# astrodeepnet/debvader

Hardware: AMD Instinct MI355X
Metric: galaxy stamps/sec (train fwd+bwd+Adam) 59x59x6 (higher is better)
Workload: dtype f32; 1 GPU; BASELINE configs[1]: 6-band 59x59 stamps, batch=256 per GPU, latent_dim=32, filters [32,64,128,256], fp32, stage-1 VAE train step; global_batch=256, per_gpu_batch=256, parallelism=dp1

## Files before the change

debvader_amd/csrc/common.h:

```cpp
#pragma once
#include <hip/hip_runtime.h>
#include <stdint.h>
#include <stddef.h>
#include <memory>
#include <utility>

namespace dv {

enum : int {
  OK = 0,
  E_INVALID = -1,
  E_HIP = -2,
  E_NOMEM = -3,
  E_RCCL = -4,
  E_STATE = -5,
  E_NODEVICE = -6,
};

void set_error(const char* fmt, ...);
int hip_fail(hipError_t e, const char* what, const char* file, int line);

#define DV_HIP(call)                                                     \
  do {                                                                   \
    hipError_t e__ = (call);                                             \
// ... 161 lines not shown
                                 const float* eps, double* res2_f = nullptr);
int launch_scene_fields_copy(double* dst_dev, const double* src_dev, const int* fptr_dev, int M, long felems, hipStream_t s);
long scene_field_mse_blocks(long felems);
int launch_scene_field_mse(const double* a_dev, const double* b_dev, const int* fptr_dev, int M, long felems,
                           double* part_dev, double* out_dev, hipStream_t s);
int launch_scene_eps_norm(const float* eps, const float* loc, int n, int cs, int nb, double* out_dev, hipStream_t s);
int launch_scene_center_mse(const double* field_dev, int F, int nb, const int* starts_dev, const float* loc, int n, int cs,
                            double* out_dev, hipStream_t s, const int* sfield_dev, int f0);
size_t scene_frac_coef_doubles(int cs, int nb, int planes);
size_t scene_frac_obj_bytes(size_t n);
int launch_scene_places(const double* dist_dev, const double* shifts_dev, int n, int F, int cs, void* objs_dev,
                        hipStream_t s);
int launch_scene_composite_frac(double* mean_f, double* std_f, double* res_f, int F, int nb, const float* loc,
                                const float* scale, const void* objs_dev, int n, int cs, hipStream_t s, const int* fptr_dev,
                                int f0, const int32_t* sfield_h, long obase, double* eps_f, const float* eps,
                                double* res2_f, double* coef_dev);
int scene_extract(const double* field_h, int F, int nb, const int32_t* starts_h, int N, int cs, double* out_h,
                  hipStream_t s);
int scene_composite(double* field_h, int F, int nb, const double* stamps_h, const double* pos_h, int N, int cs,
                    double sign, hipStream_t s);
int scene_fit_shifts(const double* field_h, int F, const double* stamps_h, int N, int cs, const double* dist_h,
                     double bound, int max_iter, double* shifts_h, double* objective_h, int32_t* iters_h,
                     int32_t* status_h, hipStream_t s);
int scene_fit_shifts_fields(const double* fields_h, int M, int F, const double* stamps_h, const int64_t* field_ptr, int N,
                            int cs, const double* dist_h, double bound, int max_iter, double* shifts_h, double* objective_h,
                            int32_t* iters_h, int32_t* status_h, size_t budget_bytes, hipStream_t s);
struct PosfitPlan;
int posfit_plan_create(int F, int cs, int N, const double* dist_h, const double* shifts_h, double bound, int max_iter,
                       PosfitPlan** out);
void posfit_plan_destroy(PosfitPlan* p);
struct PosfitPlanFree { void operator()(PosfitPlan* p) const { posfit_plan_destroy(p); } };
using PosfitPlanOwner = std::unique_ptr<PosfitPlan, PosfitPlanFree>;
int posfit_plan_layout(PosfitPlan* p, int a, int b, int max_n, const int32_t* sfield, int f0, int stamp0);
void posfit_plan_rebase(PosfitPlan* p, int a, int b, int f0);
int posfit_plan_launch_count(const PosfitPlan* p);
long posfit_plan_work_doubles(const PosfitPlan* p);
size_t posfit_plan_geom_bytes(size_t n);
int posfit_plan_upload(PosfitPlan* p, hipStream_t s);
int posfit_plan_run(const PosfitPlan* p, int l0, int l1, const double* img_dev, const double* total_sq_dev,
                    const double* stamps_dev, double* work_dev, double* shifts_dev, double* objective_dev, int* iters_dev,
                    int* status_dev, hipStream_t s);
int launch_posfit_total_sq(const double* img_dev, int nfields, long elems, double* out_dev, hipStream_t s);
int launch_posfit_band_f64(const double* src_dev, long npix, int nb, int band, double* dst_dev, hipStream_t s);
int launch_posfit_band_f32(const float* src_dev, long npix, int nb, int band, double* dst_dev, hipStream_t s);
int measure_check(const char* who, int cs, int nb, int band, double sigma0, double tol, int max_iter);
int launch_measure(const float* mean_dev, const float* stddev_dev, int n, int cs, int nb, int band, double sigma0,
                   double tol, int max_iter, double* flux_dev, double* flux_err_dev, double* shape_dev, int* iters_dev,
                   int* status_dev, hipStream_t s);
int scene_measure(const float* mean_h, const float* stddev_h, int64_t N, int cs, int nb, int band, double sigma0, double tol,
                  int max_iter, double* flux_h, double* flux_err_h, double* shape_h, int32_t* iters_h, int32_t* status_h,
                  int64_t chunk, hipStream_t s);
struct McScratch { double *flux, *shape; int *iters, *status; };
struct McState {
  double *flux_mean, *flux_std, *shape_mean, *shape_std;
  int* n_ok;
  double *sample_flux, *sample_shape;
  int* sample_status;
};
int launch_measure_mc_samples(const float* pass_dev, int rows, int cs, int nb, int band, double sigma0, double tol,
                              int max_iter, const McScratch& w, hipStream_t s);
int launch_measure_mc_fold(const McScratch& w, int n, int reps, int k0, int S, int nb, const McState& st, int64_t row0,
                           hipStream_t s);
int scene_measure_mc(const float* samples_h, int S, int64_t N, int cs, int nb, int band, double sigma0, double tol,
                     int max_iter, const McState& out_h, int64_t chunk, hipStream_t s);
int blend_check(const char* who, int cs, int nb, int band);
int launch_blend_child(const float* stamps_dev, const double* shape_dev, const int* status_dev, const int* places_dev, int n,
                       int cs, int nb, int band, int F, double* blend_dev, int* npix_dev, hipStream_t s);
int launch_blend_parent(const double* shape_dev, const int* status_dev, const int* places_dev, const int* sfield_dev, int f0,
                        int n, int cs, int nb, int band, int F, const double* model_dev, const double* data_dev,
                        double* blend_dev, hipStream_t s);
int launch_blend_composite_mean(double* mean_f, int F, int nb, const float* loc, const int* places_dev, int n, int cs,
                                const int* fptr_dev, int f0, int fy0, int nfields, long obase, hipStream_t s);
int launch_blend_set(const double* shape_dev, const int* status_dev, const int* places_dev, const int* sfield_dev, int n, int cs,
                     int nb, int band, int F, const double* mean_dev, const double* base_dev, const double* final_dev,
                     double* sums_dev, hipStream_t s);
int scene_blend(const float* stamps_h, const double* shape_h, const int32_t* status_h, const int32_t* places_h,
                const int64_t* field_ptr, int64_t N, int cs, int nb, int band, const double* model_h, const double* data_h,
                int M, int F, double* blend_h, int32_t* npix_h, int64_t chunk, int64_t gmax, hipStream_t s);
int scene_detect(const double* fields_h, int M, int H, int W, double thresh, double cont, int minarea, int nthresh,
                 int back_size, int back_filter, const double* kernel_h, int kh, int kw, int64_t workspace_bytes,
                 int64_t cap, int64_t* n_out, int64_t* offsets_h, double* globalrms_h, int32_t* field_h,
                 int32_t* parent_h, int32_t* npix_h, double* peak_h, double* flux_h, double* x_h, double* y_h,
                 double* back_h, double* rms_h, double* D_h, int32_t* labels_h, hipStream_t s);
struct DetectDevSrc {
  const double* fields_dev;
  int nb, band;
  const int32_t* which_h;
};
int scene_detect_dev(const DetectDevSrc& src, int M, int H, int W, double thresh, double cont, int minarea, int nthresh,
                     int back_size, int back_filter, const double* kernel_h, int kh, int kw, int64_t workspace_bytes,
                     int64_t cap, int64_t* n_out, int64_t* offsets_h, double* globalrms_h, int32_t* field_h,
                     int32_t* parent_h, int32_t* npix_h, double* peak_h, double* flux_h, double* x_h, double* y_h,
                     hipStream_t s);

struct GStripParams {
  const float* X;
  const float* W;
  float* U;
  float* A;
  const float* bias;
  const float* alpha;
  const float* zero;
  int NB, H, Wd, Cin, Cout;
  unsigned long long tapcode, wtcode;
  int epi;
  int R, patch_floats, strips_per_stamp, nstrips, strips_per_wg;
};
int launch_gconv_strip(GStripParams p, bool nmajor, hipStream_t s);
int launch_gconv_strip8(GStripParams p, hipStream_t s);

struct WinoParams {
  const float* X;
  const float* Ut;
  float* U;
  float* A;
  const float* bias;
  const float* alpha;
  const float* zero;
  int NB, H, Cin, Cout;
  int epi;
  int nbh, nct, NC, groups, items, items_per_wg;
};
struct WinoWDesc {
  const float* W;
  float* Ut;
  int Cin, Cout, nmajor;
  int wtmap[9];
};
struct WinoWgradParams {
  const float* X;
  const float* Y;
  float* part;
  size_t part_capacity;
  const float* zero;
  int NB, H, Cx, Cy;
  int nbh, nkt, nnt, nblocks, S, bps;
};
bool wino_wgrad_supported(int NB, int H, int Cx, int Cy);
size_t wino_wgrad_part_floats(int NB, int H, int Cx, int Cy, int* splits_out);
int launch_wino_wgrad(WinoWgradParams p, float* out, hipStream_t s);
int launch_wino_wgrad_finish(const float* part, float* out, int S, int Cx, int Cy, hipStream_t s);
bool wino_supported(int NB, int H, int Cin, int Cout);
size_t wino_weight_floats(int Cin, int Cout);
int launch_wino_weights(const WinoWDesc* descs_dev, const WinoWDesc* descs_host, int n, hipStream_t s);
int launch_wino_conv(WinoParams p, hipStream_t s);

struct GConvS2Params {
  const float* X;
  const float* W;
  float* U;
  float* A;
  const float* bias;
  const float* alpha;
  int NB, Hin, Win, Cin;
  int Hout, Wout, Cout;
  int Hc, Wc, M;
  int epi;
  int ndh[4], ndw[4];
  int cph[4], cpw[4];
  int wt[4][4];
  unsigned* dbg_out;
};
int launch_gconv_s2(const GConvS2Params& p, hipStream_t s);
void debug_set_gconv_s2_tile(int code);
void debug_set_wino_variant(int v);
void debug_set_gconv_s2_dbg(unsigned* out);

struct WGradParams {
  const float* X;
  const float* Y;
  float* part;
  int NB, Hx, Wx, Cx;
  int Hy, Wy, Cy;
  int Hc, Wc, sx, sy, ph, pw;
  int ntaps;
  TapTab xt;
  int P;
  int rows_total;
  int nsplit;
  int pchunk;
  unsigned div_hw_m, div_hw_s1, div_hw_s2, div_w_m, div_w_s1, div_w_s2;
};
int launch_wgrad(const WGradParams& p, hipStream_t s);
int launch_dense_wgrad_tn(const float* X, int ldx, const float* Y, int ldy, int NB, int I, int J, float* G, int ldg,
                          hipStream_t s);

struct WStripParams {
  const float* X;
  const float* Y;
  float* part;
  size_t part_capacity;
  int NB, Hx, Wx, Hy, Wy;
  int pb;
  const float* zero;
  int R, XR, xs_floats, ys_floats, strips_per_stamp, nstrips, strips_per_wg;
  int dbg;
  const float* U;
  const float* alpha;
  float* dal_part;
  float* db_part;
  size_t dal_capacity, db_capacity;
  long alpha_elems;
  int groups;
  int* groups_out;
};
bool wgrad_strip8_fusable(int Hy, int Wy);
void debug_set_strip(int v);
bool wgrad_strip_supported(int Cx, int Cy, int sx, int ntaps);
int launch_wgrad_strip(const WStripParams& p, int Cx, int Cy, int sx, hipStream_t s, int* nsplit_out);

#define DV_WRED_MAX 24
struct WRedEntry {
  const float* part;
  float* out;
  int nsplit, slab4, ncols4, cpad, creal;
};
struct WRedBatch {
  WRedEntry e[DV_WRED_MAX];
  int count;
};
int launch_reduce_partials_batch(const WRedBatch& b, hipStream_t s);
int launch_reduce_partials(const float* part, float* out, int nsplit, long slab_elems, int ncols, int cpad,
                           int creal, hipStream_t s);

struct HeadParams {
  const float* tpre;
  const float* y;
  const int* idx;
  int first;
  float* dt;
  float* loc;
  float* scale;
  float* part;
  int NB, Hd, H, nb, crop0;
  int ld;
  float sigma_floor;
  float gscale;
  int mse_sample;
  int mse_row0;
  unsigned mse_stream;
  unsigned long long mse_seed;
};
#define DV_MSE_STREAM 0x4D534500u
int launch_head(const HeadParams& p, hipStream_t s, int* nblocks_out);

constexpr int DV_BN_MAXC = 16;
int launch_bn_stats(const float* x, const int* idx, int first, int NB, int HW, int C, float* part, int* nblocks,
                    hipStream_t s);
int launch_reduce_rows_f64(const float* part, int nrows, int ncols, float* out, float scale, hipStream_t s,
                           int ld = 0);
int launch_bn_finalize(const float* sums, float count, int C, const float* gamma, const float* beta,
                       float* moving_mean, float* moving_var, float eps, float momentum, int unbiased,
                       int training, int update_moving, float* bnstate, hipStream_t s);
int launch_bn_apply(const float* x, const int* idx, int first, int NB, int HW, int C, int Cpad, const float* bnstate,
                    float* xn, hipStream_t s);
int launch_prelu_fwd(const float* u, const float* alpha, float* a, long NB, int E, hipStream_t s);
int launch_prelu_bwd(float* da, const float* u, const float* alpha, int NB, int E, int C, int nsplit,
                     float* dalpha_part, float* dbias_part, int* dbias_rows, hipStream_t s);
int launch_colsum(const float* x, long rows, int C, float* part, int* nrows_part, hipStream_t s);
int launch_dense_narrow(const float* x, const float* W, float* out, int NB, int K, int N, hipStream_t s);


struct SamplerParams {
  const float* t;
  float* eps;
  float* z;
  float* kl;
  float* stddev;
  int NB, d;
  int ldt, ldz;
  float diag_shift;
  int gen;
  unsigned long long seed;
  unsigned stream;
  unsigned row0;
  int rep_nb;
  const unsigned long long* seed_ptr;
  const float* slab;
  const float* tbias;
  float* t_out;
  long slab_stride;
  int nslab, lds;
  const float* alpha_in;
  float* ain;
};
int launch_sampler_fwd(const SamplerParams& p, hipStream_t s);
int launch_sampler_bwd(const float* t, const float* eps, const float* z, const float* dz, float* dt, int NB, int d,
                       int ldt, int ldz, float diag_shift, float kls, hipStream_t s);
int launch_sampler_wide_fwd(const SamplerParams& p, hipStream_t s);
int launch_sampler_wide_bwd(const float* t, const float* eps, const float* z, const float* dz, float* dt, int NB, int d,
                            int ldt, int ldz, float diag_shift, float kls, hipStream_t s);

int launch_adam(float* w, float* m, float* v, const float* g, long n, float lr_t, float b1, float b2, float eps,
                hipStream_t s);
int launch_pad_w1(const float* w, const float* gamma, const float* beta, float* wp, int taps, int cin, int cpad,
                  int cout, hipStream_t s);
int launch_bn_conv0_grads(const float* G, const float* w, const float* gamma, const float* beta, float* dW,
                          float* dgamma, float* dbeta, int taps, int cin, int cpad, int cout, hipStream_t s);
int launch_fill(float* p, long n, float v, hipStream_t s);
int launch_normalise(float* x, long n, bool inverse, hipStream_t s);
int launch_welford_update(const float* x, float* mean, float* m2, long n, int k, hipStream_t s);
int launch_welford_finish(float* m2, long n, int count, hipStream_t s);
int launch_welford_update_multi(const float* x, float* mean, float* m2, long n, int reps, int k0, hipStream_t s);
int launch_pad_cols(const float* src, float* dst, int rows, int nsrc, int ndst, hipStream_t s);
int launch_take_cols(const float* src, float* dst, int rows, int nsrc, int ndst, hipStream_t s);
int launch_gather_rows(const float* src, const int* idx, int first, int NB, long row_elems, float* dst,
                       hipStream_t s);


#if defined(__HIPCC__)
__device__ __forceinline__ void dv_dma_exec(unsigned lds, unsigned voff, const void* sbase, unsigned long long mask);
template <bool LAST16>
__device__ __forceinline__ void dv_dma_masked(unsigned lds, unsigned voff, const void* sbase, unsigned long long m_dma,
                                              unsigned vnull, const void* zero) {
// ... 27 lines not shown
```

debvader_amd/csrc/engine.hip:

```cpp
#include <rccl/rccl.h>
#include <math.h>
#include <stdarg.h>
#include <stdio.h>
#include <stdlib.h>
#include <string.h>
#include <unistd.h>

#include <algorithm>
#include <string>
#include <thread>
#include <map>
#include <memory>
#include <mutex>
#include <set>
#include <vector>
#ifdef DV_DEBUG_EXPORTS
#include <functional>
#endif

#include "../../include/debvader_hip.h"
#ifdef DV_DEBUG_EXPORTS
#include "../../include/debvader_hip_debug.h"
#endif
#include <chrono>
// ... 951 lines not shown
  p.X = X;
  p.W = W;
  p.U = U;
  p.A = Aout;
  p.bias = bias;
  p.alpha = alpha;
  p.NB = NB;
  p.Hin = p.Win = Hin;
  p.Cin = Cin;
  p.Hout = p.Wout = Hout;
  p.Cout = Cout;
  p.Hc = p.Wc = Hout;
  p.sin = s;
  p.sout = 1;
  p.ph = p.pw = 0;
  p.M = NB * Hout * Hout;
  p.w_nmajor = nmajor ? 1 : 0;
  p.epi = epi;
  Taps one;
  one.add(0, 0, 0);
  const Taps tp = single_tap ? one : taps_fprop(pb, ksz);
  const bool k3 = single_tap || ksz == 3;
  const double flops = 2.0 * NB * Hout * Hout * tp.n * (double)(W == m->W1p ? m->A.C : Cin) *
                       (double)(W == m->Whp ? 2 * m->A.C : Cout);
  if (k3 && s == 1 && pb == 1 && Hin == Hout && tp.n == 9 && !single_tap && !g_force_v1 && !g_no_special && !(fz && !m->no_fuse)) {
    const int r = wino_conv(m, X, W, nmajor, tp, bias, alpha, U, Aout, epi, NB, Hout, Cin, Cout, flops);
    if (r <= 0) return r;
  }
  if (k3 && Cin == 32 && (Cout == 16 || Cout == 32) && s == 1 && Hin == Hout && Hout >= 8 && Hout <= 64 && tp.n == 9 &&
      !single_tap && !g_force_v1 && !g_no_special && !(fz && !m->no_fuse)) {
    GStripParams g;
    memset(&g, 0, sizeof g);
    g.X = X; g.W = W; g.U = U; g.A = Aout; g.bias = bias; g.alpha = alpha; g.zero = m->zero_page;
    g.NB = NB; g.H = Hout; g.Wd = Hout; g.Cin = Cin; g.Cout = Cout;
    g.tapcode = tp.tapcode; g.wtcode = tp.wtcode; g.epi = epi;
    int r;
    {
      ProfScope ps(m, 0, nullptr, PF_GSTRIP, flops);
      r = launch_gconv_strip(g, nmajor, fwd_stream(m));
      if (r > 0) prof_uncount(m, 0, PF_GSTRIP, flops);
    }
    if (r <= 0) return r;
  }
  if (k3 && Cin == 8 && Cout == 32 && s == 1 && pb == 1 && !nmajor && Hin == Hout && Hout >= 8 && Hout <= 64 && tp.n == 9 &&
      !single_tap && !g_force_v1 && !g_no_special && !fz) {
    GStripParams g;
    memset(&g, 0, sizeof g);
    g.X = X; g.W = W; g.U = U; g.A = Aout; g.bias = bias; g.alpha = alpha; g.zero = m->zero_page;
    g.NB = NB; g.H = Hout; g.Wd = Hout; g.Cin = Cin; g.Cout = Cout; g.epi = epi;
    int r;
    {
      ProfScope ps(m, 0, nullptr, PF_GSTRIP8, flops);
      r = launch_gconv_strip8(g, fwd_stream(m));
      if (r > 0) prof_uncount(m, 0, PF_GSTRIP8, flops);
    }
    if (r <= 0) return r;
  }
  if (single_tap && nmajor && Hin == 1 && Hout == 1 && Cout <= 64 && Cin <= 1024 && epi == 0 && !bias && !fz && !g_force_v1 &&
      !g_no_special) {
    ProfScope ps(m, 2);
    if (exp_skip_small()) return OK;
    return launch_dense_narrow(X, W, U, NB, Cin, Cout, fwd_stream(m));
  }
  const bool ragged_dense = single_tap && Cin > 32 && (Cin & 3) == 0 && (Cin % 32) != 0 && !fz && !g_no_special;
  if ((Cin % 32 == 0 || ragged_dense || ((Cin == 8 || Cin == 16) && Cout <= 32 && !single_tap)) && !g_force_v1 && k3 &&
      tp.legacy) {
    GConv2Params q;
    memset(&q, 0, sizeof q);
    q.X = X; q.W = W; q.U = U; q.A = Aout; q.bias = bias; q.alpha = alpha;
    q.NB = NB; q.Hin = q.Win = Hin; q.Cin = Cin; q.Hout = q.Wout = Hout; q.Cout = Cout;
    q.sin = s; q.sout = 1; q.nclass = 1;
    q.cls[0].Hc = q.cls[0].Wc = Hout; q.cls[0].M = NB * Hout * Hout; q.cls[0].ph = q.cls[0].pw = 0;
    q.cls[0].ntaps = tp.n; q.cls[0].tapcode = tp.tapcode; q.cls[0].wtcode = tp.wtcode;
    q.w_nmajor = nmajor ? 1 : 0; q.epi = epi;
    const long MN = (long)NB * Hout * Hout * Cout;
    const long tiles64 = ((q.cls[0].M + 63) / 64) * (long)((Cout + 63) / 64);
    const int nchunks = tp.n * ((Cin + 31) / 32);
    if (single_tap && tiles64 < 256 && nchunks >= 32 && m->ws4) {
      const size_t ws4_cap = m->ws4_elems / 4;
      float* ws4 = m->ws4 + (size_t)m->lane_id * ws4_cap;
      int ks = (int)std::min<long>(std::min<long>(16, nchunks / 8), (long)(ws4_cap / (size_t)MN));
      if (ks > 1) {
        q.ksplit = ks;
        q.U = ws4;
        q.A = nullptr;
        q.epi = 0;
        {
          ProfScope ps(m, 0, nullptr, PF_GCONV2, flops);
          DV_TRY(launch_gconv2(q, fwd_stream(m)));
        }
        ProfScope ps(m, 2);
        if (exp_skip_small()) return OK;
        return launch_splitk_finish(ws4, ks, MN, Cout, epi >= 1 ? bias : nullptr, epi == 2 ? alpha : nullptr,
                                    (long)Hout * Hout * Cout, U, epi == 2 ? Aout : nullptr, fwd_stream(m));
      }
    }
    if (!fz && !single_tap) {
      const int r = gconv2_small_splitk(m, q, NB, Hout, Cout, nchunks, epi, bias, alpha, U, Aout, flops);
      if (r != 0) return r < 0 ? r : OK;
    }
    long db_rows = 0;
    const bool fuse = fz && !m->no_fuse && fuse_setup(m, q, fz, &db_rows) == OK;
    {
      ProfScope ps(m, 0, nullptr, PF_GCONV2, flops);
      DV_TRY(launch_gconv2(q, fwd_stream(m)));
    }
    if (fuse) {
      if (fused) *fused = true;
      return fuse_finish(m, q, fz, db_rows);
    }
    return OK;
  }
  fill_gconv_common(p, tp, Cin);
  ProfScope ps(m, 0, nullptr, PF_GCONV, flops);
  return launch_gconv(p, fwd_stream(m));
}

static int gconv_dgrad(dv_model* m, const float* X, const float* W, bool nmajor, const float* bias, const float* alpha,
                       float* U, float* Aout, int epi, int NB, int Hs, int Cs, int Ht, int Ct, int s, int pb,
                       const FuseBwd* fz = nullptr, bool* fused = nullptr, int ksz = 3) {
  if (fused) *fused = false;
  const double flops = 2.0 * NB * Hs * Hs * (double)(ksz * ksz) * (double)(W == m->Whp ? 2 * m->A.C : Cs) * (double)Ct;
  const bool k3 = ksz == 3;
  if (k3 && s == 1 && pb == 1 && Hs == Ht && !g_force_v1 && !g_no_special && !(fz && !m->no_fuse)) {
    const Taps tp = taps_dgrad(1, pb, 0, 0);
    if (tp.n == 9) {
      const int r = wino_conv(m, X, W, nmajor, tp, bias, alpha, U, Aout, epi, NB, Ht, Cs, Ct, flops);
      if (r <= 0) return r;
    }
  }
  if (k3 && s == 1 && (Cs == 32 || (Cs == 16 && Ct == 32)) && (Ct == 16 || Ct == 32) && Hs == Ht && Ht >= 8 && Ht <= 64 && !g_force_v1 && !g_no_special &&
      !(fz && !m->no_fuse)) {
    const Taps tp = taps_dgrad(1, pb, 0, 0);
    if (tp.n == 9) {
      GStripParams g;
      memset(&g, 0, sizeof g);
      g.X = X; g.W = W; g.U = U; g.A = Aout; g.bias = bias; g.alpha = alpha; g.zero = m->zero_page;
      g.NB = NB; g.H = Ht; g.Wd = Ht; g.Cin = Cs; g.Cout = Ct;
      g.tapcode = tp.tapcode; g.wtcode = tp.wtcode; g.epi = epi;
      int r;
      {
        ProfScope ps(m, 0, nullptr, PF_GSTRIP, flops);
        r = launch_gconv_strip(g, nmajor, fwd_stream(m));
        if (r > 0) prof_uncount(m, 0, PF_GSTRIP, flops);
      }
      if (r <= 0) return r;
    }
  }
  const bool tiny_splitk = m->tiny_call && NB <= 16 && !fz;
  if (k3 && s == 2 && Cs % 32 == 0 && Ct % 4 == 0 && nmajor && !g_force_v1 && !g_no_special && !(fz && !m->no_fuse) &&
      !tiny_splitk) {
    GConvS2Params q;
    memset(&q, 0, sizeof q);
    q.X = X; q.W = W; q.U = U; q.A = Aout; q.bias = bias; q.alpha = alpha;
    q.NB = NB; q.Hin = q.Win = Hs; q.Cin = Cs; q.Hout = q.Wout = Ht; q.Cout = Ct;
    q.Hc = q.Wc = (Ht + 1) / 2; q.M = NB * q.Hc * q.Wc; q.epi = epi;
    int two = -1, x = 0, kk[2][2] = {{-1, -1}, {-1, -1}};
    bool ok = true;
    for (int ph = 0; ph < 2; ++ph) {
      int n = 0;
      for (int kh = 0; kh < 3; ++kh) {
        const int nh = ph + pb - kh;
        if (nh & 1) continue;
        const int d = nh / 2;
        ++n;
        if (d == 0) kk[ph][0] = kh; else { kk[ph][1] = kh; x = d; two = ph; }
      }
      if (kk[ph][0] < 0 || n > 2) ok = false;
    }
    if (ok && two >= 0 && kk[1 - two][1] < 0) {
      for (int c = 0; c < 4; ++c) {
        q.cph[c] = (c & 2) ? two : 1 - two;
        q.cpw[c] = (c & 1) ? two : 1 - two;
      }
      for (int e = 0; e < 4; ++e) {
        q.ndh[e] = (e & 2) ? x : 0;
        q.ndw[e] = (e & 1) ? x : 0;
        for (int c = 0; c < 4; ++c)
          if ((e & ~c) == 0) q.wt[e][c] = kk[q.cph[c]][(e & 2) ? 1 : 0] * 3 + kk[q.cpw[c]][(e & 1) ? 1 : 0];
      }
      ProfScope ps(m, 0, nullptr, PF_GCONV_S2, flops);
      return launch_gconv_s2(q, fwd_stream(m));
    }
  }
  if (k3 && (Cs % 32 == 0 || ((Cs == 8 || Cs == 16) && Ct <= 32)) && s <= 2 && !g_force_v1) {
    GConv2Params q;
    memset(&q, 0, sizeof q);
    q.X = X; q.W = W; q.U = U; q.A = Aout; q.bias = bias; q.alpha = alpha;
    q.NB = NB; q.Hin = q.Win = Hs; q.Cin = Cs; q.Hout = q.Wout = Ht; q.Cout = Ct;
    q.sin = 1; q.sout = s; q.w_nmajor = nmajor ? 1 : 0; q.epi = epi;
    struct C { int ph, pw, n; } order[4];
    int nc = 0;
    for (int ph = 0; ph < s; ++ph)
      for (int pw = 0; pw < s; ++pw) order[nc++] = {ph, pw, taps_dgrad(s, pb, ph, pw).n};
    std::sort(order, order + nc, [](const C& a, const C& b) { return a.n > b.n; });
    int k = 0;
    for (int i = 0; i < nc; ++i) {
      int hc = (Ht - order[i].ph + s - 1) / s, wc = (Ht - order[i].pw + s - 1) / s;
      if (hc <= 0 || wc <= 0) continue;
      Taps t = taps_dgrad(s, pb, order[i].ph, order[i].pw);
      if (t.n == 0) {
        set_error("empty parity class");
        return E_INVALID;
      }
      GClass2& c = q.cls[k++];
      c.Hc = hc; c.Wc = wc; c.M = NB * hc * wc; c.ph = order[i].ph; c.pw = order[i].pw;
      c.ntaps = t.n; c.tapcode = t.tapcode; c.wtcode = t.wtcode;
    }
    q.nclass = k;
    if (!fz && k >= 1 && Cs % 32 == 0) {
      int maxtaps = 0;
      for (int i = 0; i < k; ++i) maxtaps = std::max(maxtaps, q.cls[i].ntaps);
      const int r = gconv2_small_splitk(m, q, NB, Ht, Ct, maxtaps * (Cs / 32), epi, bias, alpha, U, Aout, flops);
      if (r != 0) return r < 0 ? r : OK;
    }
    long db_rows = 0;
    const bool fuse = fz && !m->no_fuse && fuse_setup(m, q, fz, &db_rows) == OK;
    {
      ProfScope ps(m, 0, nullptr, PF_GCONV2, flops);
      DV_TRY(launch_gconv2(q, fwd_stream(m)));
    }
    if (fuse) {
      if (fused) *fused = true;
      return fuse_finish(m, q, fz, db_rows);
    }
    return OK;
  }
  for (int ph = 0; ph < s; ++ph)
    for (int pw = 0; pw < s; ++pw) {
      int hc = (Ht - ph + s - 1) / s, wc = (Ht - pw + s - 1) / s;
      if (hc <= 0 || wc <= 0) continue;
      Taps t = taps_dgrad(s, pb, ph, pw, ksz);
      GConvParams p;
      memset(&p, 0, sizeof p);
      p.X = X;
      p.W = W;
      p.U = U;
      p.A = Aout;
      p.bias = bias;
      p.alpha = alpha;
      p.NB = NB;
      p.Hin = p.Win = Hs;
      p.Cin = Cs;
      p.Hout = p.Wout = Ht;
      p.Cout = Ct;
      p.Hc = hc;
      p.Wc = wc;
      p.sin = 1;
      p.sout = s;
      p.ph = ph;
      p.pw = pw;
      p.M = NB * hc * wc;
      p.w_nmajor = nmajor ? 1 : 0;
      p.epi = epi;
      fill_gconv_common(p, t, Cs);
      ProfScope ps(m, 0, nullptr, PF_GCONV, flops * t.n / (double)(ksz * ksz));
      DV_TRY(launch_gconv(p, fwd_stream(m)));
    }
  return OK;
}

static int wgrad_impl(dv_model* m, hipStream_t ws, const float* X, int Hx, int Cx, const float* Y, int Hy, int Cy, int NB,
                      int sx, int pb, bool single_tap, float* out, int cpad, int creal, const FuseBwd* fz, int ksz);

static int wgrad(dv_model* m, const float* X, int Hx, int Cx, const float* Y, int Hy, int Cy, int NB, int sx, int pb,
                 bool single_tap, float* out, int cpad, int creal, const FuseBwd* fz = nullptr, bool on_main = false,
                 int ksz = 3) {
  hipStream_t ws = (m->wstream && !on_main) ? m->wstream : m->ctx->stream;
  if (ws != m->ctx->stream) {
    if (!m->main_marked) DV_HIP(hipEventRecord(m->ctx->ev_ready, m->ctx->stream));
    DV_HIP(hipStreamWaitEvent(ws, m->ctx->ev_ready, 0));
  }
  m->main_marked = false;
  return wgrad_impl(m, ws, X, Hx, Cx, Y, Hy, Cy, NB, sx, pb, single_tap, out, cpad, creal, fz, ksz);
}

static int wgrad_impl(dv_model* m, hipStream_t ws, const float* X, int Hx, int Cx, const float* Y, int Hy, int Cy, int NB,
                      int sx, int pb, bool single_tap, float* out, int cpad, int creal, const FuseBwd* fz, int ksz) {
  const bool k3 = ksz == 3;
  {
    static const int exp_all = DV_EXP_SWITCH("DV_EXP_SKIP_WGRAD");
    if (exp_all == 2 && !single_tap && !fz) return OK;
    if (single_tap && exp_skip_dense()) return OK;
  }
  dv_ctx* cx = m->ctx;
  const double wflops = 2.0 * NB * Hy * Hy * (single_tap ? 1.0 : (double)(ksz * ksz)) * (double)(X == m->xn ? m->A.C : Cx) *
                        (double)(out == m->Ghs ? 2 * m->A.C : Cy);
  {
    static const bool onepass = getenv("DV_DENSE_WGRAD_ONEPASS") != nullptr;
    if (single_tap && Hx == 1 && Hy == 1 && sx == 1 && cpad == creal && !fz && !g_force_v1 && !g_no_special && onepass &&
        !(Cx & 1) && !(Cy & 3)) {
      {
        ProfScope ps(m, 1, ws, PF_WGRAD, wflops);
        DV_TRY(launch_dense_wgrad_tn(X, Cx, Y, Cy, NB, Cx, Cy, out, Cy, ws));
      }
      m->ws_last_rs = ws;
      m->ws_last = -1;
      return OK;
    }
  }
  const bool rot = m->wstream && m->wstream != cx->stream && m->arena_reduce && cx->red_stream && m->ev_wk[0];
  const bool per_launch = m->ws_nreg > 3;
  float* part = m->ws1;
  size_t part_cap = m->ws1_elems;
  hipStream_t rs = ws;
  int reg = -1;
  if (rot) {
// ... 4595 lines not shown
```

debvader_amd/csrc/gconv_s2.hip:

```cpp
#include "common.h"
#include <stdlib.h>

namespace dv {

namespace {
constexpr int BKS = 32;
template <int V>
struct IC {
  static constexpr int value = V;
};
__host__ __device__ constexpr int phase_nbr(int ph) { return 3 - ph; }
__host__ __device__ constexpr int nbr_mask(int e) {
  return (e == 0) ? 15 : (e == 1) ? 10 : (e == 2) ? 12 : 8;
}
__host__ __device__ constexpr int popc4(int m) { return (m & 1) + ((m >> 1) & 1) + ((m >> 2) & 1) + ((m >> 3) & 1); }
}

template <int WGM, int WGN, int TMW = 2>
__global__ __launch_bounds__(64 * WGM * WGN) void gconv_s2_kernel(const GConvS2Params p) {
  constexpr int NW = WGM * WGN, NT = 64 * NW;
  constexpr int WMR = 16 * TMW;
  constexpr int BM = WMR * WGM, BN = 32 * WGN;
  constexpr int RP = NT / 8;
  constexpr int AROWS = BM / RP, BROWS = BN / RP;
  constexpr int A_ELEMS = BM * BKS, B_ELEMS = BN * BKS;
  constexpr int STAGE = A_ELEMS + 4 * B_ELEMS;
  constexpr int LDC = 36;
  static_assert(NW * WMR * LDC <= 2 * STAGE, "staging must fit in the operand buffers");

  extern __shared__ __attribute__((aligned(16))) float smem[];
  int* s_in = reinterpret_cast<int*>(smem + 2 * STAGE);
  int* s_nm = s_in + BM;
  int* s_out = s_nm + BM;
  int* s_al = s_out + BM;

  const unsigned long long tl0 = p.dbg_out ? __builtin_amdgcn_s_memrealtime() : 0ull;
  const int tid = threadIdx.x, lane = tid & 63, wave = tid >> 6;
  const int wm0 = (wave / WGN) * WMR, wn0 = (wave % WGN) * 32;
  const int l15 = lane & 15, lg = lane >> 4;

  int bid = blockIdx.x;
  {
    const int nwg = gridDim.x, q8 = nwg >> 3, r8 = nwg & 7, xcd = bid & 7, loc = bid >> 3;
    bid = (xcd < r8 ? xcd * (q8 + 1) : r8 * (q8 + 1) + (xcd - r8) * q8) + loc;
  }
  const int ntn = (p.Cout + BN - 1) / BN;
  const int m0 = (bid / ntn) * BM;
  const int n0 = (bid % ntn) * BN;

  if (tid < BM) {
    const int m = m0 + tid;
    int in_off = 0, nm = 0, out_off = 0, al_off = 0;
    if (m < p.M) {
      const int HW = p.Hc * p.Wc;
      const int nb = m / HW, rem = m - nb * HW;
      const int ii = rem / p.Wc, jj = rem - ii * p.Wc;
      in_off = ((nb * p.Hin + ii) * p.Win + jj) * p.Cin;
#pragma unroll
      for (int e = 0; e < 4; ++e) {
        const int ih = ii + p.ndh[e], iw = jj + p.ndw[e];
        if ((unsigned)ih < (unsigned)p.Hin && (unsigned)iw < (unsigned)p.Win) nm |= 1 << e;
      }
#pragma unroll
      for (int c = 0; c < 4; ++c)
        if (2 * ii + p.cph[c] < p.Hout && 2 * jj + p.cpw[c] < p.Wout) nm |= 16 << c;
      al_off = (2 * ii * p.Wout + 2 * jj) * p.Cout;
      out_off = nb * p.Hout * p.Wout * p.Cout + al_off;
    }
    s_in[tid] = in_off;
    s_nm[tid] = nm;
    s_out[tid] = out_off;
    s_al[tid] = al_off;
  }
  __syncthreads();

  const int kq = tid & 7, r0 = tid >> 3;
  int rin[AROWS];
  unsigned rnm = 0;
#pragma unroll
  for (int i = 0; i < AROWS; ++i) {
    rin[i] = s_in[r0 + RP * i] + kq * 4;
    rnm |= (unsigned)(s_nm[r0 + RP * i] & 15) << (4 * i);
  }
  int wthr[BROWS];
  unsigned wok = 0;
#pragma unroll
  for (int i = 0; i < BROWS; ++i) {
    const int n = n0 + r0 + RP * i;
    const bool ok = n < p.Cout;
    wthr[i] = ok ? n * p.Cin + kq * 4 : 0;
    wok |= (ok ? 1u : 0u) << i;
  }

  f32x4 areg[AROWS];
  f32x4 breg[4][BROWS];
  unsigned amask = 0;
  const int cpt = p.Cin / BKS;
  const int CC = p.Cout * p.Cin;

  auto load_global = [&](auto phase, int cc) {
    constexpr int E = phase_nbr(decltype(phase)::value);
    constexpr int MK = nbr_mask(E);
    const int tapoff = (p.ndh[E] * p.Win + p.ndw[E]) * p.Cin + cc * BKS;
    amask = 0;
#pragma unroll
    for (int i = 0; i < AROWS; ++i) {
      const bool ok = (rnm >> (4 * i + E)) & 1;
      const unsigned off = ok ? (unsigned)(rin[i] + tapoff) : 0u;
      areg[i] = *reinterpret_cast<const f32x4*>(p.X + off);
      amask |= (ok ? 1u : 0u) << i;
    }
#pragma unroll
    for (int c = 0; c < 4; ++c) {
      if ((MK >> c) & 1) {
        const int wbase = p.wt[E][c] * CC + cc * BKS;
#pragma unroll
        for (int i = 0; i < BROWS; ++i) {
          const unsigned off = ((wok >> i) & 1u) ? (unsigned)(wbase + wthr[i]) : 0u;
          breg[c][i] = *reinterpret_cast<const f32x4*>(p.W + off);
        }
      }
    }
  };

  const f32x4 zero4 = {0.f, 0.f, 0.f, 0.f};
  const int sw_w = (r0 >> 1) & 7;
  auto store_lds = [&](auto phase, int buf) {
    constexpr int MK = nbr_mask(phase_nbr(decltype(phase)::value));
    float* a = smem + buf * STAGE;
#pragma unroll
    for (int i = 0; i < AROWS; ++i)
      *reinterpret_cast<f32x4*>(a + (r0 + RP * i) * BKS + ((kq ^ sw_w) << 2)) = ((amask >> i) & 1u) ? areg[i] : zero4;
#pragma unroll
    for (int c = 0; c < 4; ++c) {
      if ((MK >> c) & 1) {
        float* b = a + A_ELEMS + c * B_ELEMS;
#pragma unroll
        for (int i = 0; i < BROWS; ++i)
          *reinterpret_cast<f32x4*>(b + (r0 + RP * i) * BKS + ((kq ^ sw_w) << 2)) = ((wok >> i) & 1u) ? breg[c][i] : zero4;
      }
    }
  };

  f32x4 acc[4][TMW][2];
#pragma unroll
  for (int c = 0; c < 4; ++c)
#pragma unroll
    for (int a = 0; a < TMW; ++a)
#pragma unroll
      for (int b = 0; b < 2; ++b) acc[c][a][b] = zero4;

  const int sw_r = l15 >> 1;
  auto compute = [&](auto phase, int buf) {
    constexpr int MK = nbr_mask(phase_nbr(decltype(phase)::value));
    const float* a = smem + buf * STAGE;
#pragma unroll
    for (int q = 0; q < 2; ++q) {
      const int quad = ((q * 4 + lg) ^ sw_r) << 2;
      f32x4 af[TMW], bf[4][2];
#pragma unroll
      for (int tm = 0; tm < TMW; ++tm) af[tm] = *reinterpret_cast<const f32x4*>(a + (wm0 + tm * 16 + l15) * BKS + quad);
#pragma unroll
      for (int c = 0; c < 4; ++c)
        if ((MK >> c) & 1) {
#pragma unroll
          for (int tn = 0; tn < 2; ++tn)
            bf[c][tn] = *reinterpret_cast<const f32x4*>(a + A_ELEMS + c * B_ELEMS + (wn0 + tn * 16 + l15) * BKS + quad);
        }
#pragma unroll
      for (int jj = 0; jj < 4; ++jj)
#pragma unroll
        for (int c = 0; c < 4; ++c)
          if ((MK >> c) & 1) {
#pragma unroll
            for (int tm = 0; tm < TMW; ++tm)
#pragma unroll
              for (int tn = 0; tn < 2; ++tn)
                acc[c][tm][tn] = __builtin_amdgcn_mfma_f32_16x16x4f32(af[tm][jj], bf[c][tn][jj], acc[c][tm][tn], 0, 0, 0);
          }
    }
  };

  auto step = [&](auto ph, auto pn, int cc_next, int cur) {
    constexpr int NMF = 16 * TMW * popc4(nbr_mask(phase_nbr(decltype(ph)::value)));
    load_global(pn, cc_next);
    compute(ph, cur);
#pragma unroll
    for (int i = 0; i < 8; ++i) {
      __builtin_amdgcn_sched_group_barrier(0x008, NMF / 8, 0);
      __builtin_amdgcn_sched_group_barrier(0x020, 2, 0);
      __builtin_amdgcn_sched_group_barrier(0x002, 10, 0);
    }
    store_lds(pn, cur ^ 1);
    __syncthreads();
  };

  int cur = 0;
  load_global(IC<0>{}, 0);
  store_lds(IC<0>{}, 0);
  __syncthreads();
  const unsigned long long tl1 = p.dbg_out ? __builtin_amdgcn_s_memrealtime() : 0ull;
  auto run_phase = [&](auto ph, auto pn, bool last) {
    for (int cc = 0; cc + 1 < cpt; ++cc) {
      step(ph, ph, cc + 1, cur);
      cur ^= 1;
    }
    if (!last) {
      step(ph, pn, 0, cur);
      cur ^= 1;
    } else {
      compute(ph, cur);
      __syncthreads();
    }
  };
  run_phase(IC<0>{}, IC<1>{}, false);
  run_phase(IC<1>{}, IC<2>{}, false);
  run_phase(IC<2>{}, IC<3>{}, false);
  run_phase(IC<3>{}, IC<3>{}, true);
  const unsigned long long tl2 = p.dbg_out ? __builtin_amdgcn_s_memrealtime() : 0ull;

  float* stg = smem + wave * (WMR * LDC);
  constexpr int RPLE = WMR / 8;
  const int f4 = lane & 7;
  const int col = n0 + wn0 + f4 * 4;
  f32x4 bias4 = {0.f, 0.f, 0.f, 0.f};
  if (p.epi >= 1 && col < p.Cout) bias4 = *reinterpret_cast<const f32x4*>(p.bias + col);
  int orow[RPLE], arow[RPLE];
  unsigned rowok = 0;
#pragma unroll
  for (int i = 0; i < RPLE; ++i) {
    const int row = wm0 + (lane >> 3) + 8 * i;
    orow[i] = s_out[row];
    arow[i] = s_al[row];
    rowok |= (unsigned)((s_nm[row] >> 4) & 15) << (4 * i);
  }
  if (col >= p.Cout) rowok = 0;
  f32x4 alr[2][RPLE];
  auto load_alpha = [&](int c, f32x4 (&dst)[RPLE]) {
    const int coff = (p.cph[c] * p.Wout + p.cpw[c]) * p.Cout;
#pragma unroll
    for (int i = 0; i < RPLE; ++i) {
      const bool ok = (rowok >> (4 * i + c)) & 1;
      dst[i] = *reinterpret_cast<const f32x4*>(p.alpha + (ok ? (unsigned)(arow[i] + coff + col) : 0u));
    }
  };
  if (p.epi == 2) load_alpha(0, alr[0]);
#pragma unroll
  for (int c = 0; c < 4; ++c) {
    if (p.epi == 2 && c + 1 < 4) load_alpha(c + 1, alr[(c + 1) & 1]);
#pragma unroll
    for (int tm = 0; tm < TMW; ++tm)
#pragma unroll
      for (int tn = 0; tn < 2; ++tn)
#pragma unroll
        for (int r = 0; r < 4; ++r) stg[(tm * 16 + lg * 4 + r) * LDC + tn * 16 + l15] = acc[c][tm][tn][r];
    __builtin_amdgcn_s_waitcnt(0xC07F);
    __builtin_amdgcn_wave_barrier();
    const int coff = (p.cph[c] * p.Wout + p.cpw[c]) * p.Cout;
#pragma unroll
    for (int i = 0; i < RPLE; ++i) {
      const int rr = (lane >> 3) + 8 * i;
      if (!((rowok >> (4 * i + c)) & 1)) continue;
      const unsigned ooff = (unsigned)(orow[i] + coff + col);
      f32x4 v = *reinterpret_cast<const f32x4*>(stg + rr * LDC + f4 * 4);
      v += bias4;
      if (p.U) *reinterpret_cast<f32x4*>(p.U + ooff) = v;
      if (p.epi == 2) {
        const f32x4 al = alr[c & 1][i];
        f32x4 o;
#pragma unroll
        for (int k = 0; k < 4; ++k) o[k] = v[k] > 0.f ? v[k] : al[k] * v[k];
        *reinterpret_cast<f32x4*>(p.A + ooff) = o;
      }
    }
    __builtin_amdgcn_wave_barrier();
  }
  if (p.dbg_out && tid == 0 && blockIdx.x < (1 << 14)) {
    __builtin_amdgcn_s_waitcnt(0);
    unsigned* d = p.dbg_out + (size_t)blockIdx.x * 4;
    d[0] = (unsigned)tl0; d[1] = (unsigned)tl1; d[2] = (unsigned)tl2; d[3] = (unsigned)__builtin_amdgcn_s_memrealtime();
  }
}

template <int WGM, int WGN, int TMW = 2>
static int launch_s2_cfg(const GConvS2Params& p, hipStream_t s) {
  constexpr int BM = 16 * TMW * WGM, BN = 32 * WGN;
  constexpr size_t smem = (size_t)2 * (BM * BKS + 4 * BN * BKS) * sizeof(float) + 4 * BM * sizeof(int);
  static bool attr_set = false;
  auto kern = gconv_s2_kernel<WGM, WGN, TMW>;
  if (!attr_set) {
    DV_HIP(hipFuncSetAttribute(reinterpret_cast<const void*>(kern), hipFuncAttributeMaxDynamicSharedMemorySize,
                               (int)smem));
    attr_set = true;
  }
  const long tiles = (long)((p.M + BM - 1) / BM) * ((p.Cout + BN - 1) / BN);
  if (tiles == 0) return OK;
  hipLaunchKernelGGL(kern, dim3((unsigned)tiles), dim3(64 * WGM * WGN), smem, s, p);
  DV_HIP(hipGetLastError());
  return OK;
}

static int s2_tile_override = -1;
void debug_set_gconv_s2_tile(int code) { s2_tile_override = code; }
static unsigned* s2_dbg_out = nullptr;
void debug_set_gconv_s2_dbg(unsigned* out) { s2_dbg_out = out; }

int launch_gconv_s2(const GConvS2Params& p0, hipStream_t s) {
  GConvS2Params p = p0;
  p.dbg_out = s2_dbg_out;
  if ((p.Cin % BKS) || (p.Cout & 3) || p.M <= 0) {
    set_error("gconv_s2: unsupported shape (Cin=%d Cout=%d M=%d)", p.Cin, p.Cout, p.M);
    return E_INVALID;
  }
  if ((long)p.NB * p.Hin * p.Win * p.Cin >= (1L << 30) || (long)p.NB * p.Hout * p.Wout * p.Cout >= (1L << 30) ||
      (long)9 * p.Cin * p.Cout >= (1L << 30)) {
    set_error("gconv_s2: tensor too large for 32-bit offsets; lower max_batch");
    return E_INVALID;
  }
  if (p.epi == 2 && (!p.alpha || !p.A)) {
    set_error("gconv_s2: PReLU epilogue needs alpha and A");
    return E_INVALID;
  }
  if (p.epi >= 1 && !p.bias) {
    set_error("gconv_s2: bias epilogue without bias");
    return E_INVALID;
  }
  int t = s2_tile_override;
  if (t < 0) {
    const long wgs128 = (long)((p.M + 127) / 128) * ((p.Cout + 31) / 32);
    t = wgs128 < 512 ? 4 : 1;
  }
  switch (t) {
    case 0: return launch_s2_cfg<2, 2>(p, s);
    case 1: return launch_s2_cfg<4, 1>(p, s);
    case 2: return launch_s2_cfg<2, 1>(p, s);
    case 4: return launch_s2_cfg<4, 1, 1>(p, s);
    default: return launch_s2_cfg<1, 2>(p, s);
  }
}

}
```

Baseline: 55480 stamps/s.

## Stream stride-2 conv operands directly to LDS via masked DMA interleaved with MFMA

The stride-2 gather conv kernel no longer stages global loads through registers and then stores them to LDS. It issues masked direct global-to-LDS loads (dv_dma_masked), with out-of-bounds rows redirected to a zero page, and spreads them across the MFMA groups of each step using sched barriers. This removes register staging and VGPR pressure and aims to overlap memory with compute. Index setup also replaces integer division with precomputed magic-number division and makes the wave index uniform via readfirstlane. The kernel now needs a zero page pointer and waits on vmcnt(0) before each barrier.

```diff
diff --git a/debvader_amd/csrc/common.h b/debvader_amd/csrc/common.h
--- a/debvader_amd/csrc/common.h
+++ b/debvader_amd/csrc/common.h
@@ -337,6 +337,7 @@
   float* A;
   const float* bias;
   const float* alpha;
+  const float* zero;
   int NB, Hin, Win, Cin;
   int Hout, Wout, Cout;
   int Hc, Wc, M;
@@ -345,6 +346,7 @@
   int cph[4], cpw[4];
   int wt[4][4];
   unsigned* dbg_out;
+  unsigned div_hw_m, div_hw_s1, div_hw_s2, div_w_m, div_w_s1, div_w_s2;
 };
 int launch_gconv_s2(const GConvS2Params& p, hipStream_t s);
 void debug_set_gconv_s2_tile(int code);
diff --git a/debvader_amd/csrc/engine.hip b/debvader_amd/csrc/engine.hip
--- a/debvader_amd/csrc/engine.hip
+++ b/debvader_amd/csrc/engine.hip
@@ -1127,7 +1127,7 @@
       !tiny_splitk) {
     GConvS2Params q;
     memset(&q, 0, sizeof q);
-    q.X = X; q.W = W; q.U = U; q.A = Aout; q.bias = bias; q.alpha = alpha;
+    q.X = X; q.W = W; q.U = U; q.A = Aout; q.bias = bias; q.alpha = alpha; q.zero = m->zero_page;
     q.NB = NB; q.Hin = q.Win = Hs; q.Cin = Cs; q.Hout = q.Wout = Ht; q.Cout = Ct;
     q.Hc = q.Wc = (Ht + 1) / 2; q.M = NB * q.Hc * q.Wc; q.epi = epi;
     int two = -1, x = 0, kk[2][2] = {{-1, -1}, {-1, -1}};
diff --git a/debvader_amd/csrc/gconv_s2.hip b/debvader_amd/csrc/gconv_s2.hip
--- a/debvader_amd/csrc/gconv_s2.hip
+++ b/debvader_amd/csrc/gconv_s2.hip
@@ -14,6 +14,15 @@
   return (e == 0) ? 15 : (e == 1) ? 10 : (e == 2) ? 12 : 8;
 }
 __host__ __device__ constexpr int popc4(int m) { return (m & 1) + ((m >> 1) & 1) + ((m >> 2) & 1) + ((m >> 3) & 1); }
+__host__ __device__ constexpr int nth_class(int m, int n) {
+  for (int c = 0; c < 4; ++c)
+    if ((m >> c) & 1) {
+      if (n == 0) return c;
+      --n;
+    }
+  return 0;
+}
+typedef __attribute__((address_space(3))) void* s2_lptr_t;
 }
 
 template <int WGM, int WGN, int TMW = 2>
@@ -35,7 +44,8 @@
   int* s_al = s_out + BM;
 
   const unsigned long long tl0 = p.dbg_out ? __builtin_amdgcn_s_memrealtime() : 0ull;
-  const int tid = threadIdx.x, lane = tid & 63, wave = tid >> 6;
+  const int tid = threadIdx.x, lane = tid & 63;
+  const int wave = __builtin_amdgcn_readfirstlane(tid >> 6);
   const int wm0 = (wave / WGN) * WMR, wn0 = (wave % WGN) * 32;
   const int l15 = lane & 15, lg = lane >> 4;
 
@@ -52,9 +62,13 @@
     const int m = m0 + tid;
     int in_off = 0, nm = 0, out_off = 0, al_off = 0;
     if (m < p.M) {
-      const int HW = p.Hc * p.Wc;
-      const int nb = m / HW, rem = m - nb * HW;
-      const int ii = rem / p.Wc, jj = rem - ii * p.Wc;
+      const unsigned um = (unsigned)m;
+      const unsigned t1 = __umulhi(p.div_hw_m, um);
+      const int nb = (int)((t1 + ((um - t1) >> p.div_hw_s1)) >> p.div_hw_s2);
+      const unsigned rem = um - (unsigned)nb * (unsigned)(p.Hc * p.Wc);
+      const unsigned t2 = __umulhi(p.div_w_m, rem);
+      const int ii = (int)((t2 + ((rem - t2) >> p.div_w_s1)) >> p.div_w_s2);
+      const int jj = (int)rem - ii * p.Wc;
       in_off = ((nb * p.Hin + ii) * p.Win + jj) * p.Cin;
 #pragma unroll
       for (int e = 0; e < 4; ++e) {
@@ -74,74 +88,55 @@
   }
   __syncthreads();
 
-  const int kq = tid & 7, r0 = tid >> 3;
-  int rin[AROWS];
-  unsigned rnm = 0;
+  const int kq = lane & 7, r0 = tid >> 3;
+  const int sw_w = (r0 >> 1) & 7;
+  const unsigned quad_b = (unsigned)((kq ^ sw_w) << 4);
+  unsigned aoff[AROWS];
+  unsigned long long am[AROWS][4];
 #pragma unroll
   for (int i = 0; i < AROWS; ++i) {
-    rin[i] = s_in[r0 + RP * i] + kq * 4;
-    rnm |= (unsigned)(s_nm[r0 + RP * i] & 15) << (4 * i);
-  }
-  int wthr[BROWS];
-  unsigned wok = 0;
+    aoff[i] = (unsigned)s_in[r0 + RP * i] * 4u + quad_b;
+    const int nmr = s_nm[r0 + RP * i];
+#pragma unroll
+    for (int e = 0; e < 4; ++e) am[i][e] = __builtin_amdgcn_ballot_w64((nmr >> e) & 1);
+  }
+  unsigned boff[BROWS];
+  unsigned long long bm[BROWS];
 #pragma unroll
   for (int i = 0; i < BROWS; ++i) {
     const int n = n0 + r0 + RP * i;
-    const bool ok = n < p.Cout;
-    wthr[i] = ok ? n * p.Cin + kq * 4 : 0;
-    wok |= (ok ? 1u : 0u) << i;
-  }
-
-  f32x4 areg[AROWS];
-  f32x4 breg[4][BROWS];
-  unsigned amask = 0;
+    boff[i] = (unsigned)(n * p.Cin) * 4u + quad_b;
+    bm[i] = __builtin_amdgcn_ballot_w64(n < p.Cout);
+  }
+  unsigned vnull = 0;
+  asm volatile("" : "+v"(vnull));
+  const int CC = p.Cout * p.Cin;
+  const char* xb[4];
+  unsigned wtb[4][4];
+#pragma unroll
+  for (int e = 0; e < 4; ++e) {
+    xb[e] = reinterpret_cast<const char*>(p.X) + (long long)((p.ndh[e] * p.Win + p.ndw[e]) * p.Cin) * 4;
+#pragma unroll
+    for (int c = 0; c < 4; ++c) wtb[e][c] = (unsigned)(p.wt[e][c] * CC) * 4u;
+  }
+  const unsigned lds0 = (unsigned)(size_t)(s2_lptr_t)smem;
+  const unsigned wrow_b = (unsigned)(wave * (8 * BKS * 4));
   const int cpt = p.Cin / BKS;
-  const int CC = p.Cout * p.Cin;
-
-  auto load_global = [&](auto phase, int cc) {
-    constexpr int E = phase_nbr(decltype(phase)::value);
+
+  auto piece = [&](auto pn, int cc, unsigned stage, int k) {
+    constexpr int E = phase_nbr(decltype(pn)::value);
     constexpr int MK = nbr_mask(E);
-    const int tapoff = (p.ndh[E] * p.Win + p.ndw[E]) * p.Cin + cc * BKS;
-    amask = 0;
-#pragma unroll
-    for (int i = 0; i < AROWS; ++i) {
-      const bool ok = (rnm >> (4 * i + E)) & 1;
-      const unsigned off = ok ? (unsigned)(rin[i] + tapoff) : 0u;
-      areg[i] = *reinterpret_cast<const f32x4*>(p.X + off);
-      amask |= (ok ? 1u : 0u) << i;
-    }
-#pragma unroll
-    for (int c = 0; c < 4; ++c) {
-      if ((MK >> c) & 1) {
-        const int wbase = p.wt[E][c] * CC + cc * BKS;
-#pragma unroll
-        for (int i = 0; i < BROWS; ++i) {
-          const unsigned off = ((wok >> i) & 1u) ? (unsigned)(wbase + wthr[i]) : 0u;
-          breg[c][i] = *reinterpret_cast<const f32x4*>(p.W + off);
-        }
-      }
+    if (k < AROWS) {
+      dv_dma_masked<false>(stage + wrow_b + k * (RP * BKS * 4), aoff[k], xb[E] + cc * (BKS * 4), am[k][E], vnull, p.zero);
+    } else {
+      const int c = nth_class(MK, (k - AROWS) / BROWS), i = (k - AROWS) % BROWS;
+      const char* base = reinterpret_cast<const char*>(p.W) + wtb[E][c] + cc * (BKS * 4);
+      dv_dma_masked<false>(stage + (A_ELEMS + c * B_ELEMS) * 4 + wrow_b + i * (RP * BKS * 4), boff[i], base, bm[i], vnull,
+                           p.zero);
     }
   };
 
   const f32x4 zero4 = {0.f, 0.f, 0.f, 0.f};
-  const int sw_w = (r0 >> 1) & 7;
-  auto store_lds = [&](auto phase, int buf) {
-    constexpr int MK = nbr_mask(phase_nbr(decltype(phase)::value));
-    float* a = smem + buf * STAGE;
-#pragma unroll
-    for (int i = 0; i < AROWS; ++i)
-      *reinterpret_cast<f32x4*>(a + (r0 + RP * i) * BKS + ((kq ^ sw_w) << 2)) = ((amask >> i) & 1u) ? areg[i] : zero4;
-#pragma unroll
-    for (int c = 0; c < 4; ++c) {
-      if ((MK >> c) & 1) {
-        float* b = a + A_ELEMS + c * B_ELEMS;
-#pragma unroll
-        for (int i = 0; i < BROWS; ++i)
-          *reinterpret_cast<f32x4*>(b + (r0 + RP * i) * BKS + ((kq ^ sw_w) << 2)) = ((wok >> i) & 1u) ? breg[c][i] : zero4;
-      }
-    }
-  };
-
   f32x4 acc[4][TMW][2];
 #pragma unroll
   for (int c = 0; c < 4; ++c)
@@ -151,72 +146,73 @@
       for (int b = 0; b < 2; ++b) acc[c][a][b] = zero4;
 
   const int sw_r = l15 >> 1;
-  auto compute = [&](auto phase, int buf) {
-    constexpr int MK = nbr_mask(phase_nbr(decltype(phase)::value));
-    const float* a = smem + buf * STAGE;
+  auto step = [&](auto ph, auto pn, auto pf, int cc_next, int cur) {
+    constexpr int MK = nbr_mask(phase_nbr(decltype(ph)::value));
+    constexpr bool PF = decltype(pf)::value != 0;
+    constexpr int NP = AROWS + popc4(nbr_mask(phase_nbr(decltype(pn)::value))) * BROWS;
+    const float* a = smem + cur * STAGE;
+    const unsigned nxt = lds0 + (unsigned)(cur ^ 1) * (STAGE * 4);
+    f32x4 af[2][TMW], bf[2][4][2];
 #pragma unroll
     for (int q = 0; q < 2; ++q) {
       const int quad = ((q * 4 + lg) ^ sw_r) << 2;
-      f32x4 af[TMW], bf[4][2];
-#pragma unroll
-      for (int tm = 0; tm < TMW; ++tm) af[tm] = *reinterpret_cast<const f32x4*>(a + (wm0 + tm * 16 + l15) * BKS + quad);
+#pragma unroll
+      for (int tm = 0; tm < TMW; ++tm) af[q][tm] = *reinterpret_cast<const f32x4*>(a + (wm0 + tm * 16 + l15) * BKS + quad);
 #pragma unroll
       for (int c = 0; c < 4; ++c)
         if ((MK >> c) & 1) {
 #pragma unroll
           for (int tn = 0; tn < 2; ++tn)
-            bf[c][tn] = *reinterpret_cast<const f32x4*>(a + A_ELEMS + c * B_ELEMS + (wn0 + tn * 16 + l15) * BKS + quad);
+            bf[q][c][tn] = *reinterpret_cast<const f32x4*>(a + A_ELEMS + c * B_ELEMS + (wn0 + tn * 16 + l15) * BKS + quad);
         }
-#pragma unroll
-      for (int jj = 0; jj < 4; ++jj)
-#pragma unroll
-        for (int c = 0; c < 4; ++c)
-          if ((MK >> c) & 1) {
-#pragma unroll
-            for (int tm = 0; tm < TMW; ++tm)
-#pragma unroll
-              for (int tn = 0; tn < 2; ++tn)
-                acc[c][tm][tn] = __builtin_amdgcn_mfma_f32_16x16x4f32(af[tm][jj], bf[c][tn][jj], acc[c][tm][tn], 0, 0, 0);
-          }
-    }
-  };
-
-  auto step = [&](auto ph, auto pn, int cc_next, int cur) {
-    constexpr int NMF = 16 * TMW * popc4(nbr_mask(phase_nbr(decltype(ph)::value)));
-    load_global(pn, cc_next);
-    compute(ph, cur);
-#pragma unroll
-    for (int i = 0; i < 8; ++i) {
-      __builtin_amdgcn_sched_group_barrier(0x008, NMF / 8, 0);
-      __builtin_amdgcn_sched_group_barrier(0x020, 2, 0);
-      __builtin_amdgcn_sched_group_barrier(0x002, 10, 0);
-    }
-    store_lds(pn, cur ^ 1);
+    }
+#pragma unroll
+    for (int g = 0; g < 8; ++g) {
+      const int q = g >> 2, jj = g & 3;
+      __builtin_amdgcn_sched_barrier(0);
+      if (PF && g < 4) {
+#pragma unroll
+        for (int k = g * NP / 4; k < (g + 1) * NP / 4; ++k) piece(pn, cc_next, nxt, k);
+      }
+#pragma unroll
+      for (int c = 0; c < 4; ++c)
+        if ((MK >> c) & 1) {
+#pragma unroll
+          for (int tm = 0; tm < TMW; ++tm)
+#pragma unroll
+            for (int tn = 0; tn < 2; ++tn)
+              acc[c][tm][tn] = __builtin_amdgcn_mfma_f32_16x16x4f32(af[q][tm][jj], bf[q][c][tn][jj], acc[c][tm][tn], 0, 0, 0);
+        }
+    }
+    asm volatile("s_waitcnt vmcnt(0)" ::: "memory");
     __syncthreads();
   };
 
   int cur = 0;
-  load_global(IC<0>{}, 0);
-  store_lds(IC<0>{}, 0);
-  __syncthreads();
+  {
+    constexpr int NP0 = AROWS + popc4(nbr_mask(phase_nbr(0))) * BROWS;
+#pragma unroll
+    for (int k = 0; k < NP0; ++k) piece(IC<0>{}, 0, lds0, k);
+    asm volatile("s_waitcnt vmcnt(0)" ::: "memory");
+    __syncthreads();
+  }
   const unsigned long long tl1 = p.dbg_out ? __builtin_amdgcn_s_memrealtime() : 0ull;
-  auto run_phase = [&](auto ph, auto pn, bool last) {
+  auto run_phase = [&](auto ph, auto pn, auto last) {
     for (int cc = 0; cc + 1 < cpt; ++cc) {
-      step(ph, ph, cc + 1, cur);
+      step(ph, ph, IC<1>{}, cc + 1, cur);
       cur ^= 1;
     }
-    if (!last) {
-      step(ph, pn, 0, cur);
+    if (!decltype(last)::value) {
+      step(ph, pn, IC<1>{}, 0, cur);
       cur ^= 1;
     } else {
-      compute(ph, cur);
-      __syncthreads();
+      step(ph, ph, IC<0>{}, 0, cur);
     }
   };
-  run_phase(IC<0>{}, IC<1>{}, false);
-  run_phase(IC<1>{}, IC<2>{}, false);
-  run_phase(IC<2>{}, IC<3>{}, false);
-  run_phase(IC<3>{}, IC<3>{}, true);
+  run_phase(IC<0>{}, IC<1>{}, IC<0>{});
+  run_phase(IC<1>{}, IC<2>{}, IC<0>{});
+  run_phase(IC<2>{}, IC<3>{}, IC<0>{});
+  run_phase(IC<3>{}, IC<3>{}, IC<1>{});
   const unsigned long long tl2 = p.dbg_out ? __builtin_amdgcn_s_memrealtime() : 0ull;
 
   float* stg = smem + wave * (WMR * LDC);
@@ -300,6 +296,14 @@
   return OK;
 }
 
+static void s2_div_consts(unsigned d, unsigned* m, unsigned* s1, unsigned* s2) {
+  unsigned l = 0;
+  while ((1ull << l) < d) ++l;
+  *m = (unsigned)((((1ull << 32) * ((1ull << l) - d)) / d) + 1);
+  *s1 = l < 1 ? l : 1;
+  *s2 = l - *s1;
+}
+
 static int s2_tile_override = -1;
 void debug_set_gconv_s2_tile(int code) { s2_tile_override = code; }
 static unsigned* s2_dbg_out = nullptr;
@@ -308,7 +312,7 @@
 int launch_gconv_s2(const GConvS2Params& p0, hipStream_t s) {
   GConvS2Params p = p0;
   p.dbg_out = s2_dbg_out;
-  if ((p.Cin % BKS) || (p.Cout & 3) || p.M <= 0) {
+  if ((p.Cin % BKS) || (p.Cout & 3) || p.M <= 0 || p.Hc < 1 || p.Wc < 1) {
     set_error("gconv_s2: unsupported shape (Cin=%d Cout=%d M=%d)", p.Cin, p.Cout, p.M);
     return E_INVALID;
   }
@@ -317,6 +321,10 @@
     set_error("gconv_s2: tensor too large for 32-bit offsets; lower max_batch");
     return E_INVALID;
   }
+  if (!p.zero) {
+    set_error("gconv_s2: no zero page");
+    return E_INVALID;
+  }
   if (p.epi == 2 && (!p.alpha || !p.A)) {
     set_error("gconv_s2: PReLU epilogue needs alpha and A");
     return E_INVALID;
@@ -325,6 +333,8 @@
     set_error("gconv_s2: bias epilogue without bias");
     return E_INVALID;
   }
+  s2_div_consts((unsigned)(p.Hc * p.Wc), &p.div_hw_m, &p.div_hw_s1, &p.div_hw_s2);
+  s2_div_consts((unsigned)p.Wc, &p.div_w_m, &p.div_w_s1, &p.div_w_s2);
   int t = s2_tile_override;
   if (t < 0) {
     const long wgs128 = (long)((p.M + 127) / 128) * ((p.Cout + 31) / 32);
```

New measurement: 55990 stamps/s, median of 6. About the same (+0.9%).
